# FuxiComputerVision/Nefii

Measured on AMD Instinct MI355X. Metric: training rays/sec (Step-2 material opt), higher is better.
Workload: dtype f16x3; 1 GPU; cfg3; parallelism=dp1, trace_tier=True, bracket_staged_eval=False, split_fp8=False, step_graph=False, cycle_batches=4, trace_prefetch=3, nonfinite_steps=0

## Files before the change

### nefii_amd/csrc/nefii_mlp.hip

```cpp
#include "mlp_tile.h"
#include "hip_check.h"

using namespace nefii;

static inline int round32(int v) { return (v + 31) & ~31; }
static inline int pad_hidden(int v) { return v <= 32 ? round32(v) : (v + 63) & ~63; }
extern "C" int nefii_padded_width(int v) { return v < 0 ? NEFII_E_ARG : pad_hidden(v); }

extern "C" int nefii_abi_version(void) { return NEFII_ABI_VERSION; }

struct PackGeom {
    int n_out, k_in, kx, ke, n_pad, x_src0, x_len, e_src0, e_len;
    float scale;
    __device__ __forceinline__ int src_col(int kk) const {
        if (kk < kx) return kk < x_len ? x_src0 + kk : -1;
        const int e = kk - kx;
        return e < e_len ? e_src0 + e : -1;
    }
    __device__ __forceinline__ float at(const float *__restrict__ W, int n, int kk) const {
        const int c = src_col(kk);
        return (n < n_out && c >= 0) ? W[(size_t)n * k_in + c] * scale : 0.f;
    }
};

// ... 611 lines not shown
    for (int j = 0; j < 8; ++j) v[j] = (_Float16)0.f;
    if (s16 < ((m.layer[l].k_x + m.layer[l].k_e) >> 4)) v = w[(((size_t)s16 * 16 + t) * 2 + part) * 64 + lane_src];
    dst[((size_t)wave * G + g) * 256 + threadIdx.x] = v;
}

__global__ void pack_mlp_stream_bwd_kernel(nefii_mlp m, half8 *__restrict__ dst, int G) {
    const int g = blockIdx.x, wave = blockIdx.y;
    int l = m.n_layers - 1, s = g;
    while (s >= mb_units(m.layer[l])) s -= mb_units(m.layer[l]), --l;
    const nefii_layer &L = m.layer[l];
    const half8 *wb = reinterpret_cast<const half8 *>(L.w_bwd_f16x3);
    const int KT = (L.k_x + L.k_e) >> 5;
    const int f = threadIdx.x >> 6, lane = threadIdx.x & 63, kg = lane >> 4;
    const int kk = 64 * wave + 16 * f + (lane & 15);
    const int s16 = 2 * s + (kg >> 1), t = kk >> 5, lane_src = (kk & 31) + 32 * (kg & 1);
    half8 v;
    for (int j = 0; j < 8; ++j) v[j] = (_Float16)0.f;
    if (s16 < (L.n_pad >> 4)) v = wb[(((size_t)s16 * KT + t) * 2) * 64 + lane_src];
    dst[((size_t)wave * G + g) * 256 + threadIdx.x] = v;
}

extern "C" int nefii_pack_mlp_stream(const nefii_mlp *h_mlp, void *w_stream, void *stream) {
    if (!h_mlp || !w_stream) return NEFII_E_ARG;
    if (nefii_mlp_stream_bytes(h_mlp) == 0) return NEFII_E_UNSUPPORTED;
    const int G = mstream_units(h_mlp);
    hipLaunchKernelGGL(pack_mlp_stream_kernel, dim3(G, 8), dim3(256), 0, (hipStream_t)stream, *h_mlp, (half8 *)w_stream, G);
    HIP_CHECK_LAUNCH();
    const int Gb = mstream_units_bwd(h_mlp);
    if (Gb > 0) {
        hipLaunchKernelGGL(pack_mlp_stream_bwd_kernel, dim3(Gb, 8), dim3(256), 0, (hipStream_t)stream, *h_mlp,
                           (half8 *)w_stream + (size_t)8 * G * 256, Gb);
        HIP_CHECK_LAUNCH();
    }
    return 0;
}

template <int QT, int EW, bool H16>
__global__ __launch_bounds__(512, 2) void mlp_forward16q_kernel(nefii_mlp m, const float *__restrict__ in_a,
                                                               const float *__restrict__ in_b,
                                                               const float *__restrict__ in_c,
                                                               const float *__restrict__ feat, int64_t n,
                                                               float *__restrict__ out, int out_stride,
                                                               float *__restrict__ hidden_out, int hid_stride,
                                                               void *__restrict__ stash_v, int stash_stride,
                                                               float *__restrict__ z_last, _Float16 *__restrict__ x0_16, int G) {
    NEFII_CLAIM_SIMD_2();
    float *const stash = H16 ? nullptr : static_cast<float *>(stash_v);
    _Float16 *const stash16 = H16 ? static_cast<_Float16 *>(stash_v) : nullptr;
    constexpr int ROWS = 16 * QT, XP = LdsM<QT, EW>::XP, EP = 512, NW = 8, NJ = 4 * QT, RT = (QT + 1) / 2;
    __shared__ LdsM<QT, EW> lds;
    __shared__ float raw[ROWS * 9];
    const int tid = threadIdx.x;
    const int wave = __builtin_amdgcn_readfirstlane(tid >> 6), lane = tid & 63;
    const int NH = m.n_layers - 1;
    const float inv_scale = 1.f / (W16_SCALE * A16_SCALE);
    const int64_t n_tiles = (n + ROWS - 1) / ROWS;
    {
        uint32_t *z = reinterpret_cast<uint32_t *>(&lds);
        for (int i = tid; i < (int)(sizeof(lds) / 4); i += 512) z[i] = 0u;
    }
    P16<8>::Stage b[4];
    PCursor cur;
    cur.bytes = (unsigned)G * 4096;
    cur.base = reinterpret_cast<const half8 *>(m.w_stream) + (size_t)wave * G * 256 + lane;
    cur.off = 0;
#pragma unroll
    for (int u = 0; u < 3; ++u) pload<8>(b[u], cur);
    const int boff = 64 * wave + lane;
    const _Float16 *qh0 = lds.Xh + (lane & 15) * XP + 8 * (lane >> 4), *ql0 = lds.Xl + (lane & 15) * XP + 8 * (lane >> 4);
    const int w0 = enc_width(m.enc_freqs[0]), w1 = enc_width(m.enc_freqs[1]), w2 = enc_width(m.enc_freqs[2]);
    const int F = m.feat_width, kx0 = m.layer[0].k_x;
    __syncthreads();
    for (int64_t tile = blockIdx.x; tile < n_tiles; tile += gridDim.x) {
        const int64_t base = tile * ROWS;
        for (int i = tid; i < ROWS * 9; i += 512) {
            const int p = i / 9, c = i - 9 * p, which = c / 3;
            const float *src = which == 0 ? in_a : (which == 1 ? in_b : in_c);
            int64_t idx = base + p;
            if (idx >= n) idx = n - 1;
            raw[i] = (src && m.enc_freqs[which] >= 0) ? src[idx * 3 + (c - 3 * which)] : 0.f;
        }
        if (feat && F == kx0 && (F & 3) == 0 && (reinterpret_cast<uintptr_t>(feat) & 15) == 0) {
            const int q4 = kx0 >> 2;
            for (int i = tid; i < ROWS * q4; i += 512) {
                const int p = i / q4, f = 4 * (i - p * q4);
                int64_t idx = base + p;
                if (idx >= n) idx = n - 1;
                const float4v v = *reinterpret_cast<const float4v *>(feat + idx * F + f) * A16_SCALE;
                const half4 hi = __builtin_convertvector(v, half4);
                *reinterpret_cast<half4 *>(lds.Xh + p * XP + EP - kx0 + f) = hi;
                *reinterpret_cast<half4 *>(lds.Xl + p * XP + EP - kx0 + f) =
                    __builtin_convertvector(v - __builtin_convertvector(hi, float4v), half4);
            }
        } else {
            for (int i = tid; i < ROWS * kx0; i += 512) {
                const int p = i / kx0, f = i - p * kx0;
                int64_t idx = base + p;
                if (idx >= n) idx = n - 1;
                const float v = (feat && f < F) ? feat[idx * F + f] : 0.f;
                split16a(v, lds.Xh[p * XP + EP - kx0 + f], lds.Xl[p * XP + EP - kx0 + f]);
            }
        }
        float bnext = m.layer[0].bias[boff];
        __syncthreads();
        for (int i = tid; i < ROWS * EW; i += 512) {
            const int p = i / EW, c = i - p * EW;
            float val = 0.f;
            if (c < w0) val = enc_value(raw + p * 9, c);
            else if (c < w0 + w1) val = enc_value(raw + p * 9 + 3, c - w0);
            else if (c < w0 + w1 + w2) val = enc_value(raw + p * 9 + 6, c - w0 - w1);
            split16a(val, lds.Xh[p * XP + EP + c], lds.Xl[p * XP + EP + c]);
        }
        __syncthreads();
        if (H16 && x0_16) {
            const int C = (kx0 + EW) >> 3;
            for (int i = tid; i < ROWS * C; i += 512) {
                const int p = i / C, c = i - p * C;
                if (base + p < n)
                    *reinterpret_cast<half8 *>(x0_16 + (size_t)(base + p) * (kx0 + EW) + 8 * c) =
                        *reinterpret_cast<const half8 *>(lds.Xh + p * XP + EP - kx0 + 8 * c);
            }
        }
        for (int l = 0; l < NH; ++l) {
            const nefii_layer &L = m.layer[l];
            const int units = m_units(L);
            const _Float16 *ah = qh0 + (EP - L.k_x), *al = ql0 + (EP - L.k_x);
            const float *bp = m.layer[l + 1 < NH ? l + 1 : l].bias + boff;
            asm volatile("" ::"s"(units), "v"(ah), "v"(al), "v"(bp));
            __builtin_amdgcn_s_waitcnt(0x0070);
            __builtin_amdgcn_sched_barrier(0);
            const float bvec = bnext;
            f32x4 acc[NJ];
#pragma unroll
            for (int j = 0; j < NJ; ++j)
#pragma unroll
                for (int i = 0; i < 4; ++i) acc[j][i] = 0.f;
            QAct<QT> a[2];
            qload_a<QT, XP>(a[0], ah, al, 0);
            qgemm<QT, 4, XP>(units, b, a, cur, ah, al, acc);
            bnext = *bp;
            __builtin_amdgcn_sched_barrier(0);
            half4 phi[NJ], plo[NJ];
            const int bsrc = __builtin_bit_cast(int, bvec);
            const bool pre_last = hidden_out != nullptr && l == NH - 1;
            auto epilogue = [&](auto actc) {
                constexpr int ACT = decltype(actc)::value;
#pragma unroll
                for (int ft = 0; ft < 4; ++ft) {
                    float4v bs;
#pragma unroll
                    for (int k = 0; k < 4; ++k)
                        bs[k] = __builtin_bit_cast(float, __builtin_amdgcn_ds_bpermute(4 * (16 * ft + 4 * (lane >> 4) + k), bsrc));
                    const int f0 = 64 * wave + 16 * ft + 4 * (lane >> 4);
#pragma unroll
                    for (int qt = 0; qt < QT; ++qt) {
                        const int j = ft * QT + qt;
                        float4v hv;
#pragma unroll
                        for (int k = 0; k < 4; ++k) {
                            const float z = __builtin_fmaf(acc[j][k], inv_scale, bs[k]);
                            hv[k] = ACT == NEFII_ACT_ELU ? elu_fast(z) : act_fwd(z, ACT);
                        }
                        const int64_t row = base + 16 * qt + (lane & 15);
                        if (row < n) {
                            if (stash) *reinterpret_cast<float4v *>(stash + ((size_t)l * n + row) * stash_stride + f0) = hv;
                            if (pre_last) {
#pragma unroll
                                for (int k = 0; k < 4; ++k)
                                    if (f0 + k < L.n_out) hidden_out[(size_t)row * hid_stride + f0 + k] = hv[k];
                            }
                        }
                        const float4v hs = hv * A16_SCALE;
                        const half4 hi = __builtin_convertvector(hs, half4);
                        phi[j] = hi;
                        plo[j] = __builtin_convertvector(hs - __builtin_convertvector(hi, float4v), half4);
// ... 71 lines not shown
            __syncthreads();
        }
    }
}

static int check_mlp16(const nefii_mlp *m, bool bwd) {
    int rc = check_mlp(m, false);
    if (rc) return rc;
    for (int l = 0; l < m->n_layers; ++l) {
        if (!m->layer[l].w_f16x3) return NEFII_E_ARG;
        if (bwd && l > 0 && !m->layer[l].w_bwd_f16x3) return NEFII_E_ARG;
        if ((m->layer[l].k_x | m->layer[l].k_e | m->layer[l].n_pad) & 15) return NEFII_E_SHAPE;
    }
    return 0;
}

static bool mlp_stream_enabled() {
    static const bool v = env_int("NEFII_MLP_STREAM", 1) != 0;
    return v;
}
static bool mlp_streams_both_ways(const nefii_mlp *m) {
    return m->w_stream && mlp_stream_enabled() && mstream_shape(m) && mstream_units_bwd(m) > 0;
}
static dim3 stream_grid(int64_t n) {
    const int64_t t = (n + 63) / 64;
    return dim3((int)(t < 256 ? t : 256));
}

template <bool H16>
static int launch_forward16q(const nefii_mlp *h_mlp, const float *in_a, const float *in_b, const float *in_c, const float *feat,
                             int64_t n, float *out, int out_stride, float *hidden_out, int hid_stride, void *stash,
                             int stash_stride, float *z_last, void *x0_16, void *stream) {
    const auto kernel = mstream_shape(h_mlp) == 64 ? mlp_forward16q_kernel<4, 64, H16> : mlp_forward16q_kernel<4, 96, H16>;
    hipLaunchKernelGGL(kernel, stream_grid(n), dim3(512), 0, (hipStream_t)stream, *h_mlp, in_a, in_b, in_c, feat, n, out,
                       out_stride, hidden_out, hid_stride, stash, stash_stride, z_last, (_Float16 *)x0_16, mstream_units(h_mlp));
    HIP_CHECK_LAUNCH();
    return 0;
}

extern "C" int nefii_mlp_forward_f16(const nefii_mlp *h_mlp, const float *in_a, const float *in_b, const float *in_c,
                                     const float *feat, int64_t n, float *out, int out_stride, float *hidden_out,
                                     int hid_stride, float *stash, int stash_stride, int single_pass, void *stream) {
    int rc = check_mlp16(h_mlp, false);
    if (rc) return rc;
    if (n <= 0) return 0;
    if (!out) return NEFII_E_ARG;
    const int64_t n_tiles = (n + TILE - 1) / TILE;
    if (!single_pass && h_mlp->w_stream && mlp_stream_enabled() && mstream_shape(h_mlp))
        return launch_forward16q<false>(h_mlp, in_a, in_b, in_c, feat, n, out, out_stride, hidden_out, hid_stride, stash,
                                        stash_stride, nullptr, nullptr, stream);
    if (single_pass)
        hipLaunchKernelGGL(mlp_forward16_kernel<true>, dim3(grid_for(n_tiles, 1)), dim3(WG), 0, (hipStream_t)stream, *h_mlp,
                           in_a, in_b, in_c, feat, n, out, out_stride, hidden_out, hid_stride, stash, stash_stride);
    else
        hipLaunchKernelGGL(mlp_forward16_kernel<false>, dim3(grid_for(n_tiles, 1)), dim3(WG), 0, (hipStream_t)stream, *h_mlp,
                           in_a, in_b, in_c, feat, n, out, out_stride, hidden_out, hid_stride, stash, stash_stride);
    HIP_CHECK_LAUNCH();
    return 0;
}

extern "C" int nefii_mlp_h16_supported(const nefii_mlp *h_mlp) {
    if (!h_mlp || check_mlp16(h_mlp, true)) return 0;
    return mlp_streams_both_ways(h_mlp);
}

extern "C" int nefii_mlp_x0_width(const nefii_mlp *h_mlp) {
    if (!nefii_mlp_h16_supported(h_mlp)) return 0;
    return h_mlp->layer[0].k_x + mstream_shape(h_mlp);
}

extern "C" int nefii_mlp_forward_f16h(const nefii_mlp *h_mlp, const float *in_a, const float *in_b, const float *in_c,
                                      const float *feat, int64_t n, float *out, int out_stride, float *hidden_out,
                                      int hid_stride, void *stash16, int stash_stride, float *z_last, void *x0_16,
                                      void *stream) {
    int rc = check_mlp16(h_mlp, false);
    if (rc) return rc;
    if (!nefii_mlp_h16_supported(h_mlp)) return NEFII_E_SHAPE;
    if (n <= 0) return 0;
    if (!out || !stash16 || !z_last || (stash_stride & 3)) return NEFII_E_ARG;
    return launch_forward16q<true>(h_mlp, in_a, in_b, in_c, feat, n, out, out_stride, hidden_out, hid_stride, stash16,
                                   stash_stride, z_last, x0_16, stream);
}

__global__ void grad_scale_kernel(const float *__restrict__ d, int64_t count, float *__restrict__ scale) {
    __shared__ float wmax[16];
    float mx = 0.f;
    for (int64_t i = threadIdx.x; i < count; i += blockDim.x) {
        const float v = fabsf(d[i]);
        mx = (v < 3.0e38f && v > mx) ? v : mx;
    }
#pragma unroll
    for (int o = 32; o > 0; o >>= 1) mx = fmaxf(mx, __shfl_xor(mx, o));
    if ((threadIdx.x & 63) == 0) wmax[threadIdx.x >> 6] = mx;
    __syncthreads();
    if (threadIdx.x == 0) {
        for (int w = 1; w < (int)(blockDim.x >> 6); ++w) mx = fmaxf(mx, wmax[w]);
        float s = 1.f;
        if (mx > 0.f) {
            int e;
            frexpf(mx, &e);
            e = 8 - e;
            e = e < -40 ? -40 : (e > 60 ? 60 : e);
            s = ldexpf(1.f, e);
        }
        scale[0] = s;
    }
}

__global__ void grad_scale_head_kernel(const float *__restrict__ d, int out_stride, const float *__restrict__ pre, int pre_stride,
                                       int64_t n, int n_out, int head, float *__restrict__ scale) {
    __shared__ float wmax[16];
    float mx = 0.f;
    const int64_t count = n * n_out;
    for (int64_t i = threadIdx.x; i < count; i += blockDim.x) {
        const int64_t p = i / n_out;
        const int c = (int)(i - p * n_out);
        const float dv = d[p * out_stride + c], z = pre[p * pre_stride + c];
        const float v = fabsf(dv);
        const float hv = fabsf(dv * head_bwd_from_out(head_fwd(z, head), z, head)) * 0.125f;
        mx = (v < 3.0e38f && v > mx) ? v : mx;
        mx = (hv < 3.0e38f && hv > mx) ? hv : mx;
    }
#pragma unroll
    for (int o = 32; o > 0; o >>= 1) mx = fmaxf(mx, __shfl_xor(mx, o));
    if ((threadIdx.x & 63) == 0) wmax[threadIdx.x >> 6] = mx;
    __syncthreads();
    if (threadIdx.x == 0) {
        for (int w = 1; w < (int)(blockDim.x >> 6); ++w) mx = fmaxf(mx, wmax[w]);
        float s = 1.f;
        if (mx > 0.f) {
            int e;
            frexpf(mx, &e);
            e = 8 - e;
            e = e < -40 ? -40 : (e > 60 ? 60 : e);
            s = ldexpf(1.f, e);
        }
        scale[0] = s;
    }
}

extern "C" int nefii_mlp_grad_scale_head(const float *d_out, int out_stride, const float *pre, int pre_stride, int64_t n,
                                         int n_out, int head, float *scale, void *stream) {
    if (!d_out || !pre || !scale || n < 0 || n_out < 1 || out_stride < n_out || pre_stride < n_out) return NEFII_E_ARG;
    if (head < NEFII_HEAD_NONE || head > NEFII_HEAD_RELU_INIT) return NEFII_E_ARG;
    hipLaunchKernelGGL(grad_scale_head_kernel, dim3(1), dim3(1024), 0, (hipStream_t)stream, d_out, out_stride, pre, pre_stride, n,
                       n_out, head, scale);
    HIP_CHECK_LAUNCH();
    return 0;
}

extern "C" int nefii_mlp_grad_scale(const float *d_out, int64_t count, float *scale, void *stream) {
    if (!d_out || !scale || count < 0) return NEFII_E_ARG;
    hipLaunchKernelGGL(grad_scale_kernel, dim3(1), dim3(1024), 0, (hipStream_t)stream, d_out, count, scale);
    HIP_CHECK_LAUNCH();
    return 0;
}

__global__ __launch_bounds__(256, 2) void mlp_backward16_kernel(nefii_mlp m, const float *__restrict__ d_out,
                                                                int out_stride, const float *__restrict__ stash,
                                                                int stash_stride, int64_t n, float *__restrict__ dz,
                                                                int dz_stride, const float *__restrict__ scale) {
    __shared__ _Float16 Xh[TILE * XS16];
    const int tid = threadIdx.x;
    const int Lm1 = m.n_layers - 1;
    const float S = scale[0];
    const float inv = 1.f / (W16_SCALE * S);
    const int64_t n_tiles = (n + TILE - 1) / TILE;
    for (int64_t tile = blockIdx.x; tile < n_tiles; tile += gridDim.x) {
        const int64_t base = tile * TILE;
        {
            const nefii_layer &L = m.layer[Lm1];
            for (int i = tid; i < TILE * L.n_pad; i += WG) {
                const int p = i / L.n_pad, c = i - p * L.n_pad;
                float v = 0.f;
                if (base + p < n && c < L.n_out) {
                    const float pre = stash[((size_t)Lm1 * n + base + p) * stash_stride + c];
                    const float y = head_fwd(pre, m.head);
                    v = d_out[(size_t)(base + p) * out_stride + c] * head_bwd_from_out(y, pre, m.head);
                }
                Xh[p * XS16 + c] = (_Float16)(v * S);
                if (base + p < n) dz[((size_t)Lm1 * n + base + p) * dz_stride + c] = v;
            }
        }
        __syncthreads();
        for (int l = Lm1; l >= 1; --l) {
            const nefii_layer &L = m.layer[l];
            f32x16 acc[4];
            const int wave = __builtin_amdgcn_readfirstlane(tid >> 6), lane = tid & 63;
            const int NTs = (L.k_x + L.k_e) >> 5, ntc = L.k_x >> 5;
            int ntw = (ntc - wave + 3) >> 2;
            if (ntw < 0) ntw = 0;
            zero_acc(acc);
            gemm_block16<true>(Xh, Xh, XS16, L.n_pad >> 4, reinterpret_cast<const half8 *>(L.w_bwd_f16x3), NTs, wave, lane,
                               ntw, acc);
            __syncthreads();
            NEFII_ACT_SWITCH(m.act, {
                NEFII_FOR_ACC(acc, ntw, {
                    const bool live = (base + row) < n;
                    float v = 0.f;
                    if (live) {
                        const float hprev = stash[((size_t)(l - 1) * n + base + row) * stash_stride + col];
                        v = val * inv * act_bwd_from_out(hprev, ACT);
                        dz[((size_t)(l - 1) * n + base + row) * dz_stride + col] = v;
                    }
                    Xh[row * XS16 + col] = (_Float16)(v * S);
                })
            })
            __syncthreads();
        }
    }
}

template <bool H16>
__global__ __launch_bounds__(512, 2) void mlp_backward16s_kernel(nefii_mlp m, const float *__restrict__ d_out, int out_stride,
                                                                const void *__restrict__ stash_v, int stash_stride,
                                                                const float *__restrict__ z_last, int64_t n,
                                                                void *__restrict__ dz_v, int dz_stride,
                                                                const float *__restrict__ scale, size_t stream_off, int G) {
    NEFII_CLAIM_SIMD_2();
    const float *const stash = static_cast<const float *>(stash_v);
    const _Float16 *const stash16 = static_cast<const _Float16 *>(stash_v);
    float *const dz = static_cast<float *>(dz_v);
    _Float16 *const dz16 = static_cast<_Float16 *>(dz_v);
    constexpr int QT = 4, FT = 4, ROWS = 64, XP = QGeo<4>::XP, NJ = FT * QT;
    __shared__ LdsS<4, ROWS> lds;
    const int tid = threadIdx.x;
    const int wave = __builtin_amdgcn_readfirstlane(tid >> 6), lane = tid & 63;
    const int Lm1 = m.n_layers - 1;
    const float S = scale[0];
    const float inv = 1.f / (W16_SCALE * S);
    const int64_t n_tiles = (n + ROWS - 1) / ROWS;
    {
        uint32_t *z = reinterpret_cast<uint32_t *>(&lds);
        for (int i = tid; i < (int)(sizeof(lds) / 4); i += 512) z[i] = 0u;
    }
    SStage<4> b[4];
    PCursor cur;
    cur.bytes = (unsigned)G * 4096;
    cur.base = reinterpret_cast<const half8 *>(m.w_stream) + stream_off + (size_t)wave * G * 256 + lane;
    cur.off = 0;
#pragma unroll
    for (int u = 0; u < 3; ++u) sload<4>(b[u], cur);
    const _Float16 *qh0 = lds.Xh + (lane & 15) * XP + 8 * (lane >> 4);
    __syncthreads();
    for (int64_t tile = blockIdx.x; tile < n_tiles; tile += gridDim.x) {
        const int64_t base = tile * ROWS;
        {
            const nefii_layer &L = m.layer[Lm1];
            const int kpad = mb_units(L) * 32;
            for (int i = tid; i < ROWS * kpad; i += 512) {
                const int p = i / kpad, c = i - p * kpad;
                float v = 0.f;
                if (base + p < n && c < L.n_pad) {
                    if (c < L.n_out) {
                        const float pre = H16 ? z_last[(size_t)(base + p) * 8 + c]
                                              : stash[((size_t)Lm1 * n + base + p) * stash_stride + c];
                        const float y = head_fwd(pre, m.head);
                        v = d_out[(size_t)(base + p) * out_stride + c] * head_bwd_from_out(y, pre, m.head);
                    }
                    if (H16) dz16[((size_t)Lm1 * n + base + p) * dz_stride + c] = (_Float16)(v * S);
                    else dz[((size_t)Lm1 * n + base + p) * dz_stride + c] = v;
                }
                lds.Xh[p * XP + c] = (_Float16)(v * S);
            }
        }
        __syncthreads();
        for (int l = Lm1; l >= 1; --l) {
            const nefii_layer &L = m.layer[l];
            const int units = mb_units(L);
            asm volatile("" ::"s"(units));
            __builtin_amdgcn_s_waitcnt(0x0070);
            __builtin_amdgcn_sched_barrier(0);
            f32x4 acc[NJ];
#pragma unroll
            for (int j = 0; j < NJ; ++j)
#pragma unroll
                for (int i = 0; i < 4; ++i) acc[j][i] = 0.f;
            SAct<QT> a[2];
            sload_a<QT, XP>(a[0], qh0, 0);
            sgemm<QT, FT, true>(units, b, a, cur, qh0, acc);
            half4 phi[NJ];
            const float *sp = stash + (size_t)(l - 1) * n * stash_stride;
            float *dp = dz + (size_t)(l - 1) * n * dz_stride;
            const _Float16 *sp16 = stash16 + (size_t)(l - 1) * n * stash_stride;
            _Float16 *dp16 = dz16 + (size_t)(l - 1) * n * dz_stride;
            auto epilogue = [&](auto actc) {
                constexpr int ACT = decltype(actc)::value;
#pragma unroll
                for (int ft = 0; ft < FT; ++ft) {
                    const int f0 = 64 * wave + 16 * ft + 4 * (lane >> 4);
#pragma unroll
                    for (int qt = 0; qt < QT; ++qt) {
                        const int j = ft * QT + qt;
                        const int64_t row = base + 16 * qt + (lane & 15);
                        float4v v = {0.f, 0.f, 0.f, 0.f};
                        if (row < n) {
                            float4v h;
                            if (H16)
                                h = __builtin_convertvector(*reinterpret_cast<const half4 *>(sp16 + (size_t)row * stash_stride + f0),
                                                            float4v) * (1.f / A16_SCALE);
                            else
                                h = *reinterpret_cast<const float4v *>(sp + (size_t)row * stash_stride + f0);
#pragma unroll
                            for (int k = 0; k < 4; ++k) v[k] = acc[j][k] * inv * act_bwd_from_out(h[k], ACT);
                            if (!H16) *reinterpret_cast<float4v *>(dp + (size_t)row * dz_stride + f0) = v;
                        }
                        phi[j] = __builtin_convertvector(v * S, half4);
                        if (H16 && row < n) *reinterpret_cast<half4 *>(dp16 + (size_t)row * dz_stride + f0) = phi[j];
                    }
                }
            };
            if (m.act == NEFII_ACT_RELU)
                epilogue(std::integral_constant<int, NEFII_ACT_RELU>{});
            else if (m.act == NEFII_ACT_ELU)
                epilogue(std::integral_constant<int, NEFII_ACT_ELU>{});
            else
                epilogue(std::integral_constant<int, NEFII_ACT_SOFTPLUS100>{});
            __syncthreads();
#pragma unroll
            for (int ft = 0; ft < FT; ++ft) {
                const int f0 = 64 * wave + 16 * ft + 4 * (lane >> 4);
#pragma unroll
                for (int qt = 0; qt < QT; ++qt)
                    *reinterpret_cast<half4 *>(lds.Xh + (16 * qt + (lane & 15)) * XP + f0) = phi[ft * QT + qt];
            }
            __syncthreads();
        }
    }
}

template <bool H16>
static int launch_backward16s(const nefii_mlp *h_mlp, const float *d_out, int out_stride, const void *stash, int stash_stride,
                              const float *z_last, int64_t n, void *dz, int dz_stride, const float *scale, void *stream) {
    hipLaunchKernelGGL(mlp_backward16s_kernel<H16>, stream_grid(n), dim3(512), 0, (hipStream_t)stream, *h_mlp, d_out, out_stride,
                       stash, stash_stride, z_last, n, dz, dz_stride, scale, (size_t)8 * mstream_units(h_mlp) * 256,
                       mstream_units_bwd(h_mlp));
    HIP_CHECK_LAUNCH();
    return 0;
}

extern "C" int nefii_mlp_backward_f16(const nefii_mlp *h_mlp, const float *d_out, int out_stride, const float *stash,
                                      int stash_stride, int64_t n, float *dz, int dz_stride, const float *scale,
                                      void *stream) {
    int rc = check_mlp16(h_mlp, true);
    if (rc) return rc;
    if (n <= 0) return 0;
    if (!d_out || !stash || !dz || !scale) return NEFII_E_ARG;
    if (mlp_streams_both_ways(h_mlp) && (stash_stride & 3) == 0 && (dz_stride & 3) == 0)
        return launch_backward16s<false>(h_mlp, d_out, out_stride, stash, stash_stride, nullptr, n, dz, dz_stride, scale, stream);
    const int64_t n_tiles = (n + TILE - 1) / TILE;
    hipLaunchKernelGGL(mlp_backward16_kernel, dim3(grid_for(n_tiles, 2)), dim3(WG), 0, (hipStream_t)stream, *h_mlp, d_out,
                       out_stride, stash, stash_stride, n, dz, dz_stride, scale);
    HIP_CHECK_LAUNCH();
    return 0;
}

extern "C" int nefii_mlp_backward_f16h(const nefii_mlp *h_mlp, const float *d_out, int out_stride, const void *stash16,
                                       int stash_stride, const float *z_last, int64_t n, void *dz16, int dz_stride,
                                       const float *scale, void *stream) {
    int rc = check_mlp16(h_mlp, true);
    if (rc) return rc;
    if (!nefii_mlp_h16_supported(h_mlp)) return NEFII_E_SHAPE;
    if (n <= 0) return 0;
    if (!d_out || !stash16 || !z_last || !dz16 || !scale || (stash_stride & 3) || (dz_stride & 3)) return NEFII_E_ARG;
    return launch_backward16s<true>(h_mlp, d_out, out_stride, stash16, stash_stride, z_last, n, dz16, dz_stride, scale, stream);
}

template <bool DZ16, bool X16>
__device__ __forceinline__ void wgrad16_body(const void *__restrict__ dz_v, int dz_stride, const void *__restrict__ x_v,
                                             int x_stride, int64_t P, int n_out, int k_in, float scale,
                                             const float *__restrict__ gscale, float *__restrict__ dW, float *__restrict__ db,
                                             int atomic, int bx, int by, int bz, int gz) {
    const float *const dz = static_cast<const float *>(dz_v), *const x = static_cast<const float *>(x_v);
    const _Float16 *const dz16 = static_cast<const _Float16 *>(dz_v), *const x16 = static_cast<const _Float16 *>(x_v);
    const int wave = threadIdx.x >> 6, lane = threadIdx.x & 63;
    const int i = lane & 31, h = lane >> 5;
    const int n0 = bx * 64 + (wave & 1) * 32;
    const int k0 = by * 256 + (wave >> 1) * 128;
    const int64_t chunk = ((P + gz - 1) / gz + 15) & ~(int64_t)15;
    const int64_t p_begin = (int64_t)bz * chunk;
    const int64_t p_end = p_begin + chunk < P ? p_begin + chunk : P;
    const float S = gscale[0];
    f32x16 acc[4];
    zero_acc(acc);
    const bool n_ok = (n0 + i) < n_out;
    bool k_ok[4];
#pragma unroll
    for (int t = 0; t < 4; ++t) k_ok[t] = (k0 + 32 * t + i) < k_in;
    float bsum = 0.f;
    if (n0 < n_out && k0 < k_in) {
        const int nc = n_ok ? n0 + i : n_out - 1;
// ... 122 lines not shown
                    for (int e = 0; e < 8; ++e) a[e] = na + e < n_out ? a[e] : (_Float16)0;
                }
                ha[u] = pr < p_end ? a : hzero;
            }
        } else {
#pragma unroll
            for (int u = 0; u < 4; ++u) {
                const int64_t pr = pb + r8 + 8 * u;
                const int64_t pc = pr < p_end ? pr : p_end - 1;
                float4v a = {0.f, 0.f, 0.f, 0.f};
                if (n_in) {
                    a = *reinterpret_cast<const float4v *>(dz + pc * dz_stride + na);
                } else {
#pragma unroll
                    for (int e = 0; e < 4; ++e) a[e] = dz[pc * dz_stride + (na + e < n_out ? na + e : n_out - 1)];
#pragma unroll
                    for (int e = 0; e < 4; ++e) a[e] = na + e < n_out ? a[e] : 0.f;
                }
                ra[u] = pr < p_end ? a : float4v{0.f, 0.f, 0.f, 0.f};
            }
        }
        if (X16) {
#pragma unroll
            for (int u = 0; u < 2; ++u) {
                const int64_t pr = pb + r16 + 16 * u;
                const int64_t pc = pr < p_end ? pr : p_end - 1;
                half8 b = hzero;
                if (XVEC && k_in_ok) {
                    b = *reinterpret_cast<const half8 *>(x16 + pc * x_stride + ka);
                } else {
#pragma unroll
                    for (int e = 0; e < 8; ++e) b[e] = x16[pc * x_stride + (ka + e < k_in ? ka + e : k_in - 1)];
#pragma unroll
                    for (int e = 0; e < 8; ++e) b[e] = ka + e < k_in ? b[e] : (_Float16)0;
                }
                hb[u] = pr < p_end ? b : hzero;
            }
        } else {
#pragma unroll
            for (int u = 0; u < 4; ++u) {
                const int64_t pr = pb + r8 + 8 * u;
                const int64_t pc = pr < p_end ? pr : p_end - 1;
                float4v b = {0.f, 0.f, 0.f, 0.f};
                if (XVEC && k_in_ok) {
                    b = *reinterpret_cast<const float4v *>(x + pc * x_stride + ka);
                } else {
#pragma unroll
                    for (int e = 0; e < 4; ++e) b[e] = x[pc * x_stride + (ka + e < k_in ? ka + e : k_in - 1)];
#pragma unroll
                    for (int e = 0; e < 4; ++e) b[e] = ka + e < k_in ? b[e] : 0.f;
                }
                rb[u] = pr < p_end ? b : float4v{0.f, 0.f, 0.f, 0.f};
            }
        }
    };
    auto stage = [&](int buf) {
        if (DZ16) {
#pragma unroll
            for (int u = 0; u < 2; ++u) {
#pragma unroll
                for (int e = 0; e < 8; ++e) bsum[e] += (float)ha[u][e];
                *reinterpret_cast<half8 *>(&A[buf][(r16 + 16 * u) * WG2_STRIDE + 8 * c8]) = ha[u];
            }
        } else {
#pragma unroll
            for (int u = 0; u < 4; ++u) {
#pragma unroll
                for (int e = 0; e < 4; ++e) bsum[e] += ra[u][e];
                *reinterpret_cast<half4 *>(&A[buf][(r8 + 8 * u) * WG2_STRIDE + 4 * c4]) = __builtin_convertvector(ra[u] * S, half4);
            }
        }
        if (X16) {
#pragma unroll
            for (int u = 0; u < 2; ++u) *reinterpret_cast<half8 *>(&B[buf][(r16 + 16 * u) * WG2_STRIDE + 8 * c8]) = hb[u];
        } else {
#pragma unroll
            for (int u = 0; u < 4; ++u)
                *reinterpret_cast<half4 *>(&B[buf][(r8 + 8 * u) * WG2_STRIDE + 4 * c4]) = __builtin_convertvector(rb[u], half4);
        }
    };
    f32x16 acc[4];
    zero_acc(acc);
    const int an = 64 * (wave & 1), bk = 64 * (wave >> 1);
    fetch(p_begin);
    stage(0);
    __syncthreads();
    int buf = 0;
    for (int64_t pb = p_begin; pb < p_end; pb += WG2_ROWS) {
        const bool more = pb + WG2_ROWS < p_end;
        if (more) fetch(pb + WG2_ROWS);
#pragma unroll
        for (int ks = 0; ks < 2; ++ks) {
            half8 af[2], bf[2];
#pragma unroll
            for (int t = 0; t < 2; ++t) {
                af[t] = wg2_fragment(A[buf], an + 32 * t, 16 * ks, lane);
                bf[t] = wg2_fragment(B[buf], bk + 32 * t, 16 * ks, lane);
            }
#pragma unroll
            for (int t = 0; t < 2; ++t)
#pragma unroll
                for (int v = 0; v < 2; ++v)
                    acc[2 * t + v] = __builtin_amdgcn_mfma_f32_32x32x16_f16(af[t], bf[v], acc[2 * t + v], 0, 0, 0);
        }
        if (more) stage(buf ^ 1);
        __syncthreads();
        buf ^= 1;
    }
    const float os = scale / S * (X16 ? 1.f / A16_SCALE : 1.f);
    const int i = lane & 31, h = lane >> 5;
#pragma unroll
    for (int t = 0; t < 2; ++t)
#pragma unroll
        for (int v = 0; v < 2; ++v)
#pragma unroll
            for (int r = 0; r < 16; ++r) {
                const int nn = n0 + an + 32 * t + (r & 3) + 8 * (r >> 2) + 4 * h, k = k0 + bk + 32 * v + i;
                if (nn < n_out && k < k_in) atomicAdd(&dW[(size_t)nn * k_in + k], acc[2 * t + v][r] * os);
            }
    if (db && tk == 0) {
        __syncthreads();
        float *red = reinterpret_cast<float *>(&A[0][0]);
        if (DZ16) {
#pragma unroll
            for (int e = 0; e < 8; ++e) red[r16 * 128 + 8 * c8 + e] = bsum[e];
        } else {
#pragma unroll
            for (int e = 0; e < 4; ++e) red[r8 * 128 + 4 * c4 + e] = bsum[e];
        }
        __syncthreads();
        if (tid < 128 && n0 + tid < n_out) {
            float sum = 0.f;
#pragma unroll
            for (int g = 0; g < (DZ16 ? 16 : 8); ++g) sum += red[g * 128 + tid];
            atomicAdd(&db[n0 + tid], DZ16 ? sum / S : sum);
        }
    }
}

template <bool XVEC, bool DZ16, bool X16>
__global__ __launch_bounds__(256, 2) void mlp_wgrad16t_kernel(const void *__restrict__ dz_v, int dz_stride,
                                                              const void *__restrict__ x_v, int x_stride, int64_t P, int n_out,
                                                              int k_in, float scale, const float *__restrict__ gscale,
                                                              float *__restrict__ dW, float *__restrict__ db, int splits,
                                                              int tiles_n, int tiles_k) {
    wgrad16t_body<XVEC, DZ16, X16>(dz_v, dz_stride, x_v, x_stride, P, n_out, k_in, scale, gscale, dW, db, splits, tiles_n, tiles_k,
                                   blockIdx.x);
}

struct WgradBatch {
    nefii_wgrad_item it[NEFII_MAX_WGRAD_ITEMS];
    unsigned first[NEFII_MAX_WGRAD_ITEMS + 1];
    int aux0[NEFII_MAX_WGRAD_ITEMS], aux1[NEFII_MAX_WGRAD_ITEMS], aux2[NEFII_MAX_WGRAD_ITEMS];
    int n;
};
__device__ __forceinline__ int wgrad_batch_item(const WgradBatch &b, unsigned bid) {
    int i = 0;
    while (i + 1 < b.n && bid >= b.first[i + 1]) ++i;
    return __builtin_amdgcn_readfirstlane(i);
}
template <bool XVEC, bool X16>
__global__ __launch_bounds__(256, 2) void mlp_wgrad16t_batch_kernel(WgradBatch b, int64_t P, const float *__restrict__ gscale) {
    const int i = wgrad_batch_item(b, blockIdx.x);
    const nefii_wgrad_item &w = b.it[i];
    wgrad16t_body<XVEC, true, X16>(w.dz16, w.dz_stride, w.x, w.x_stride, P, w.n_out, w.k_in, w.scale, gscale, w.dW, w.db, b.aux0[i],
                                   b.aux1[i], b.aux2[i], blockIdx.x - b.first[i]);
}
template <bool X16>
__global__ __launch_bounds__(256) void mlp_wgrad16_batch_kernel(WgradBatch b, int64_t P, const float *__restrict__ gscale) {
    const int i = wgrad_batch_item(b, blockIdx.x);
    const nefii_wgrad_item &w = b.it[i];
    const int local = blockIdx.x - b.first[i], gx = b.aux0[i], gy = b.aux1[i], gz = b.aux2[i];
    wgrad16_body<true, X16>(w.dz16, w.dz_stride, w.x, w.x_stride, P, w.n_out, w.k_in, w.scale, gscale, w.dW, w.db, gz > 1 ? 1 : 0,
                            local % gx, (local / gx) % gy, local / (gx * gy), gz);
}
__global__ void zero_fill_batch_kernel(WgradBatch b) {
    const int i = wgrad_batch_item(b, blockIdx.x);
    const nefii_wgrad_item &w = b.it[i];
    const size_t e = (size_t)(blockIdx.x - b.first[i]) * blockDim.x + threadIdx.x, nw = (size_t)w.n_out * w.k_in;
    if (e < nw) w.dW[e] = 0.f;
    else if (w.db && e - nw < (size_t)w.n_out) w.db[e - nw] = 0.f;
}

static bool wgrad_tr_enabled() {
    static const bool v = env_int("NEFII_WGRAD_TR", 1) != 0;
    return v;
}

struct WgradPlan {
    bool blocked, xvec, needs_zero_fill;
// ... 359 lines not shown
```

Measured before the change: 2.009 million rays/s.

## Batch loads in MLP kernels, parallelize grad-scale, deepen weight-grad prefetch

Several independent changes. The feature-load loop issues four vector loads before converting them. The grad-scale reductions become a multi-block reduction using atomicMax plus clear and finish kernels when the input is large. The backward head and activation epilogues are restructured to issue stash loads up front with clamped rows. The weight-gradient GEMM gains a two-stage register prefetch path for full 128x128 fp16 tiles. Together these aim to expose more memory-level parallelism and to stop a single block from serializing the reduction, at the cost of more registers and extra kernel launches.

```diff
diff --git a/nefii_amd/csrc/nefii_mlp.hip b/nefii_amd/csrc/nefii_mlp.hip
--- a/nefii_amd/csrc/nefii_mlp.hip
+++ b/nefii_amd/csrc/nefii_mlp.hip
@@ -717,15 +717,29 @@
         }
         if (feat && F == kx0 && (F & 3) == 0 && (reinterpret_cast<uintptr_t>(feat) & 15) == 0) {
             const int q4 = kx0 >> 2;
-            for (int i = tid; i < ROWS * q4; i += 512) {
-                const int p = i / q4, f = 4 * (i - p * q4);
-                int64_t idx = base + p;
-                if (idx >= n) idx = n - 1;
-                const float4v v = *reinterpret_cast<const float4v *>(feat + idx * F + f) * A16_SCALE;
-                const half4 hi = __builtin_convertvector(v, half4);
-                *reinterpret_cast<half4 *>(lds.Xh + p * XP + EP - kx0 + f) = hi;
-                *reinterpret_cast<half4 *>(lds.Xl + p * XP + EP - kx0 + f) =
-                    __builtin_convertvector(v - __builtin_convertvector(hi, float4v), half4);
+            constexpr int FG = 4;
+            for (int i0 = tid; i0 < ROWS * q4; i0 += FG * 512) {
+                float4v v[FG];
+#pragma unroll
+                for (int u = 0; u < FG; ++u) {
+                    const int i = i0 + u * 512 < ROWS * q4 ? i0 + u * 512 : ROWS * q4 - 1;
+                    const int p = i / q4, f = 4 * (i - p * q4);
+                    int64_t idx = base + p;
+                    if (idx >= n) idx = n - 1;
+                    v[u] = *reinterpret_cast<const float4v *>(feat + idx * F + f);
+                }
+#pragma unroll
+                for (int u = 0; u < FG; ++u) {
+                    const int i = i0 + u * 512;
+                    if (i < ROWS * q4) {
+                        const int p = i / q4, f = 4 * (i - p * q4);
+                        const float4v w = v[u] * A16_SCALE;
+                        const half4 hi = __builtin_convertvector(w, half4);
+                        *reinterpret_cast<half4 *>(lds.Xh + p * XP + EP - kx0 + f) = hi;
+                        *reinterpret_cast<half4 *>(lds.Xl + p * XP + EP - kx0 + f) =
+                            __builtin_convertvector(w - __builtin_convertvector(hi, float4v), half4);
+                    }
+                }
             }
         } else {
             for (int i = tid; i < ROWS * kx0; i += 512) {
@@ -963,6 +977,17 @@
                                    stash_stride, z_last, x0_16, stream);
 }
 
+__device__ __forceinline__ float gs_from_max(float mx) {
+    float s = 1.f;
+    if (mx > 0.f) {
+        int e;
+        frexpf(mx, &e);
+        e = 8 - e;
+        e = e < -40 ? -40 : (e > 60 ? 60 : e);
+        s = ldexpf(1.f, e);
+    }
+    return s;
+}
 __global__ void grad_scale_kernel(const float *__restrict__ d, int64_t count, float *__restrict__ scale) {
     __shared__ float wmax[16];
     float mx = 0.f;
@@ -976,15 +1001,7 @@
     __syncthreads();
     if (threadIdx.x == 0) {
         for (int w = 1; w < (int)(blockDim.x >> 6); ++w) mx = fmaxf(mx, wmax[w]);
-        float s = 1.f;
-        if (mx > 0.f) {
-            int e;
-            frexpf(mx, &e);
-            e = 8 - e;
-            e = e < -40 ? -40 : (e > 60 ? 60 : e);
-            s = ldexpf(1.f, e);
-        }
-        scale[0] = s;
+        scale[0] = gs_from_max(mx);
     }
 }
 
@@ -1008,31 +1025,135 @@
     __syncthreads();
     if (threadIdx.x == 0) {
         for (int w = 1; w < (int)(blockDim.x >> 6); ++w) mx = fmaxf(mx, wmax[w]);
-        float s = 1.f;
-        if (mx > 0.f) {
-            int e;
-            frexpf(mx, &e);
-            e = 8 - e;
-            e = e < -40 ? -40 : (e > 60 ? 60 : e);
-            s = ldexpf(1.f, e);
-        }
-        scale[0] = s;
-    }
+        scale[0] = gs_from_max(mx);
+    }
+}
+
+constexpr int64_t GS_ONE_BLOCK = 65536;
+constexpr int GS_WG = 256, GS_U = 4;
+
+__device__ __forceinline__ float gs_fold(float mx, float v) {
+    return (v < 3.0e38f && v > mx) ? v : mx;
+}
+__device__ __forceinline__ void gs_block_max(float mx, float *__restrict__ scale) {
+    __shared__ float wmax[GS_WG / 64];
+#pragma unroll
+    for (int o = 32; o > 0; o >>= 1) mx = fmaxf(mx, __shfl_xor(mx, o));
+    if ((threadIdx.x & 63) == 0) wmax[threadIdx.x >> 6] = mx;
+    __syncthreads();
+    if (threadIdx.x == 0) {
+#pragma unroll
+        for (int w = 1; w < GS_WG / 64; ++w) mx = fmaxf(mx, wmax[w]);
+        if (mx > 0.f) atomicMax(reinterpret_cast<unsigned *>(scale), __float_as_uint(mx));
+    }
+}
+__global__ void grad_scale_clear_kernel(float *__restrict__ scale) { scale[0] = 0.f; }
+__global__ void grad_scale_finish_kernel(float *__restrict__ scale) { scale[0] = gs_from_max(scale[0]); }
+
+template <bool VEC>
+__global__ __launch_bounds__(GS_WG) void grad_scale_blocks_kernel(const float *__restrict__ d, int64_t count,
+                                                                  float *__restrict__ scale) {
+    float mx = 0.f;
+    const int64_t stride = (int64_t)gridDim.x * GS_WG;
+    const int64_t t = (int64_t)blockIdx.x * GS_WG + threadIdx.x;
+    if (VEC) {
+        const int64_t quads = count >> 2;
+        const float4v *d4 = reinterpret_cast<const float4v *>(d);
+        for (int64_t i = t; i < quads; i += GS_U * stride) {
+            float4v v[GS_U];
+#pragma unroll
+            for (int u = 0; u < GS_U; ++u) {
+                const int64_t k = i + u * stride;
+                v[u] = d4[k < quads ? k : quads - 1];
+            }
+#pragma unroll
+            for (int u = 0; u < GS_U; ++u)
+#pragma unroll
+                for (int e = 0; e < 4; ++e) mx = gs_fold(mx, fabsf(v[u][e]));
+        }
+        if (blockIdx.x == 0 && threadIdx.x < (count & 3)) mx = gs_fold(mx, fabsf(d[(quads << 2) + threadIdx.x]));
+    } else {
+        for (int64_t i = t; i < count; i += GS_U * stride) {
+            float v[GS_U];
+#pragma unroll
+            for (int u = 0; u < GS_U; ++u) {
+                const int64_t k = i + u * stride;
+                v[u] = d[k < count ? k : count - 1];
+            }
+#pragma unroll
+            for (int u = 0; u < GS_U; ++u) mx = gs_fold(mx, fabsf(v[u]));
+        }
+    }
+    gs_block_max(mx, scale);
+}
+
+__global__ __launch_bounds__(GS_WG) void grad_scale_head_blocks_kernel(const float *__restrict__ d, int out_stride,
+                                                                       const float *__restrict__ pre, int pre_stride, int64_t n,
+                                                                       int n_out, int head, float *__restrict__ scale) {
+    float mx = 0.f;
+    const int64_t count = n * n_out;
+    const int64_t stride = (int64_t)gridDim.x * GS_WG;
+    for (int64_t i = (int64_t)blockIdx.x * GS_WG + threadIdx.x; i < count; i += GS_U * stride) {
+        float dv[GS_U], z[GS_U];
+#pragma unroll
+        for (int u = 0; u < GS_U; ++u) {
+            const int64_t k = i + u * stride, kc = k < count ? k : count - 1;
+            const int64_t p = kc / n_out;
+            const int c = (int)(kc - p * n_out);
+            dv[u] = d[p * out_stride + c];
+            z[u] = pre[p * pre_stride + c];
+        }
+#pragma unroll
+        for (int u = 0; u < GS_U; ++u) {
+            mx = gs_fold(mx, fabsf(dv[u]));
+            mx = gs_fold(mx, fabsf(dv[u] * head_bwd_from_out(head_fwd(z[u], head), z[u], head)) * 0.125f);
+        }
+    }
+    gs_block_max(mx, scale);
+}
+
+static int gs_grid(int64_t units) {
+    const int64_t g = (units + (int64_t)GS_WG * GS_U - 1) / ((int64_t)GS_WG * GS_U);
+    return (int)(g < 1 ? 1 : (g > 2048 ? 2048 : g));
 }
 
 extern "C" int nefii_mlp_grad_scale_head(const float *d_out, int out_stride, const float *pre, int pre_stride, int64_t n,
                                          int n_out, int head, float *scale, void *stream) {
     if (!d_out || !pre || !scale || n < 0 || n_out < 1 || out_stride < n_out || pre_stride < n_out) return NEFII_E_ARG;
     if (head < NEFII_HEAD_NONE || head > NEFII_HEAD_RELU_INIT) return NEFII_E_ARG;
-    hipLaunchKernelGGL(grad_scale_head_kernel, dim3(1), dim3(1024), 0, (hipStream_t)stream, d_out, out_stride, pre, pre_stride, n,
-                       n_out, head, scale);
+    hipStream_t st = (hipStream_t)stream;
+    if (n * n_out <= GS_ONE_BLOCK) {
+        hipLaunchKernelGGL(grad_scale_head_kernel, dim3(1), dim3(1024), 0, st, d_out, out_stride, pre, pre_stride, n, n_out, head,
+                           scale);
+        HIP_CHECK_LAUNCH();
+        return 0;
+    }
+    hipLaunchKernelGGL(grad_scale_clear_kernel, dim3(1), dim3(1), 0, st, scale);
+    HIP_CHECK_LAUNCH();
+    hipLaunchKernelGGL(grad_scale_head_blocks_kernel, dim3(gs_grid(n * n_out)), dim3(GS_WG), 0, st, d_out, out_stride, pre,
+                       pre_stride, n, n_out, head, scale);
+    HIP_CHECK_LAUNCH();
+    hipLaunchKernelGGL(grad_scale_finish_kernel, dim3(1), dim3(1), 0, st, scale);
     HIP_CHECK_LAUNCH();
     return 0;
 }
 
 extern "C" int nefii_mlp_grad_scale(const float *d_out, int64_t count, float *scale, void *stream) {
     if (!d_out || !scale || count < 0) return NEFII_E_ARG;
-    hipLaunchKernelGGL(grad_scale_kernel, dim3(1), dim3(1024), 0, (hipStream_t)stream, d_out, count, scale);
+    hipStream_t st = (hipStream_t)stream;
+    if (count <= GS_ONE_BLOCK) {
+        hipLaunchKernelGGL(grad_scale_kernel, dim3(1), dim3(1024), 0, st, d_out, count, scale);
+        HIP_CHECK_LAUNCH();
+        return 0;
+    }
+    hipLaunchKernelGGL(grad_scale_clear_kernel, dim3(1), dim3(1), 0, st, scale);
+    HIP_CHECK_LAUNCH();
+    if ((reinterpret_cast<uintptr_t>(d_out) & 15) == 0)
+        hipLaunchKernelGGL(grad_scale_blocks_kernel<true>, dim3(gs_grid(count >> 2)), dim3(GS_WG), 0, st, d_out, count, scale);
+    else
+        hipLaunchKernelGGL(grad_scale_blocks_kernel<false>, dim3(gs_grid(count)), dim3(GS_WG), 0, st, d_out, count, scale);
+    HIP_CHECK_LAUNCH();
+    hipLaunchKernelGGL(grad_scale_finish_kernel, dim3(1), dim3(1), 0, st, scale);
     HIP_CHECK_LAUNCH();
     return 0;
 }
@@ -1129,18 +1250,29 @@
         {
             const nefii_layer &L = m.layer[Lm1];
             const int kpad = mb_units(L) * 32;
+            const int n_out = L.n_out;
             for (int i = tid; i < ROWS * kpad; i += 512) {
                 const int p = i / kpad, c = i - p * kpad;
-                float v = 0.f;
-                if (base + p < n && c < L.n_pad) {
-                    if (c < L.n_out) {
-                        const float pre = H16 ? z_last[(size_t)(base + p) * 8 + c]
-                                              : stash[((size_t)Lm1 * n + base + p) * stash_stride + c];
-                        const float y = head_fwd(pre, m.head);
-                        v = d_out[(size_t)(base + p) * out_stride + c] * head_bwd_from_out(y, pre, m.head);
+                if (c >= n_out) {
+                    lds.Xh[p * XP + c] = (_Float16)0.f;
+                    if (base + p < n && c < L.n_pad) {
+                        if (H16) dz16[((size_t)Lm1 * n + base + p) * dz_stride + c] = (_Float16)0.f;
+                        else dz[((size_t)Lm1 * n + base + p) * dz_stride + c] = 0.f;
                     }
-                    if (H16) dz16[((size_t)Lm1 * n + base + p) * dz_stride + c] = (_Float16)(v * S);
-                    else dz[((size_t)Lm1 * n + base + p) * dz_stride + c] = v;
+                }
+            }
+            for (int i = tid; i < ROWS * n_out; i += 512) {
+                const int p = i / n_out, c = i - p * n_out;
+                const bool live = base + p < n;
+                const int64_t rc = live ? base + p : n - 1;
+                const float pre = H16 ? z_last[(size_t)rc * 8 + c] : stash[((size_t)Lm1 * n + rc) * stash_stride + c];
+                const float dv = d_out[(size_t)rc * out_stride + c];
+                const float y = head_fwd(pre, m.head);
+                const float g = dv * head_bwd_from_out(y, pre, m.head);
+                const float v = live ? g : 0.f;
+                if (live) {
+                    if (H16) dz16[((size_t)Lm1 * n + rc) * dz_stride + c] = (_Float16)(v * S);
+                    else dz[((size_t)Lm1 * n + rc) * dz_stride + c] = v;
                 }
                 lds.Xh[p * XP + c] = (_Float16)(v * S);
             }
@@ -1165,29 +1297,61 @@
             float *dp = dz + (size_t)(l - 1) * n * dz_stride;
             const _Float16 *sp16 = stash16 + (size_t)(l - 1) * n * stash_stride;
             _Float16 *dp16 = dz16 + (size_t)(l - 1) * n * dz_stride;
+            bool live[QT];
+            size_t srow[QT];
+#pragma unroll
+            for (int qt = 0; qt < QT; ++qt) {
+                const int64_t row = base + 16 * qt + (lane & 15);
+                live[qt] = row < n;
+                srow[qt] = (size_t)(live[qt] ? row : n - 1) * stash_stride + 64 * wave + 4 * (lane >> 4);
+            }
             auto epilogue = [&](auto actc) {
                 constexpr int ACT = decltype(actc)::value;
-#pragma unroll
-                for (int ft = 0; ft < FT; ++ft) {
-                    const int f0 = 64 * wave + 16 * ft + 4 * (lane >> 4);
-#pragma unroll
-                    for (int qt = 0; qt < QT; ++qt) {
-                        const int j = ft * QT + qt;
-                        const int64_t row = base + 16 * qt + (lane & 15);
-                        float4v v = {0.f, 0.f, 0.f, 0.f};
-                        if (row < n) {
-                            float4v h;
-                            if (H16)
-                                h = __builtin_convertvector(*reinterpret_cast<const half4 *>(sp16 + (size_t)row * stash_stride + f0),
-                                                            float4v) * (1.f / A16_SCALE);
-                            else
-                                h = *reinterpret_cast<const float4v *>(sp + (size_t)row * stash_stride + f0);
-#pragma unroll
-                            for (int k = 0; k < 4; ++k) v[k] = acc[j][k] * inv * act_bwd_from_out(h[k], ACT);
-                            if (!H16) *reinterpret_cast<float4v *>(dp + (size_t)row * dz_stride + f0) = v;
+                if constexpr (H16) {
+                    half4 hs[NJ];
+#pragma unroll
+                    for (int ft = 0; ft < FT; ++ft)
+#pragma unroll
+                        for (int qt = 0; qt < QT; ++qt)
+                            hs[ft * QT + qt] = *reinterpret_cast<const half4 *>(sp16 + srow[qt] + 16 * ft);
+#pragma unroll
+                    for (int ft = 0; ft < FT; ++ft)
+#pragma unroll
+                        for (int qt = 0; qt < QT; ++qt) {
+                            const int j = ft * QT + qt;
+                            const float4v h = __builtin_convertvector(hs[j], float4v) * (1.f / A16_SCALE);
+                            float4v v;
+#pragma unroll
+                            for (int k = 0; k < 4; ++k) v[k] = live[qt] ? acc[j][k] * inv * act_bwd_from_out(h[k], ACT) : 0.f;
+                            phi[j] = __builtin_convertvector(v * S, half4);
                         }
-                        phi[j] = __builtin_convertvector(v * S, half4);
-                        if (H16 && row < n) *reinterpret_cast<half4 *>(dp16 + (size_t)row * dz_stride + f0) = phi[j];
+#pragma unroll
+                    for (int qt = 0; qt < QT; ++qt)
+                        if (live[qt]) {
+                            _Float16 *drow = dp16 + (size_t)(base + 16 * qt + (lane & 15)) * dz_stride + 64 * wave + 4 * (lane >> 4);
+#pragma unroll
+                            for (int ft = 0; ft < FT; ++ft) *reinterpret_cast<half4 *>(drow + 16 * ft) = phi[ft * QT + qt];
+                        }
+                } else {
+#pragma unroll
+                    for (int ft = 0; ft < FT; ++ft) {
+                        float4v hs[QT];
+#pragma unroll
+                        for (int qt = 0; qt < QT; ++qt) hs[qt] = *reinterpret_cast<const float4v *>(sp + srow[qt] + 16 * ft);
+#pragma unroll
+                        for (int qt = 0; qt < QT; ++qt) {
+                            const int j = ft * QT + qt;
+                            float4v v;
+#pragma unroll
+                            for (int k = 0; k < 4; ++k) v[k] = live[qt] ? acc[j][k] * inv * act_bwd_from_out(hs[qt][k], ACT) : 0.f;
+                            hs[qt] = v;
+                            phi[j] = __builtin_convertvector(v * S, half4);
+                        }
+#pragma unroll
+                        for (int qt = 0; qt < QT; ++qt)
+                            if (live[qt])
+                                *reinterpret_cast<float4v *>(dp + (size_t)(base + 16 * qt + (lane & 15)) * dz_stride + 64 * wave +
+                                                             4 * (lane >> 4) + 16 * ft) = hs[qt];
                     }
                 }
             };
@@ -1476,13 +1640,7 @@
     f32x16 acc[4];
     zero_acc(acc);
     const int an = 64 * (wave & 1), bk = 64 * (wave >> 1);
-    fetch(p_begin);
-    stage(0);
-    __syncthreads();
-    int buf = 0;
-    for (int64_t pb = p_begin; pb < p_end; pb += WG2_ROWS) {
-        const bool more = pb + WG2_ROWS < p_end;
-        if (more) fetch(pb + WG2_ROWS);
+    auto products = [&](int buf) {
 #pragma unroll
         for (int ks = 0; ks < 2; ++ks) {
             half8 af[2], bf[2];
@@ -1497,9 +1655,64 @@
                 for (int v = 0; v < 2; ++v)
                     acc[2 * t + v] = __builtin_amdgcn_mfma_f32_32x32x16_f16(af[t], bf[v], acc[2 * t + v], 0, 0, 0);
         }
-        if (more) stage(buf ^ 1);
+    };
+    bool done = false;
+    if constexpr (XVEC && DZ16 && X16) {
+        if (n0 + 128 <= n_out && k0 + 128 <= k_in) {
+            half8 qa[2][2], qb[2][2];
+            auto fetch2 = [&](int s, int64_t pb) {
+#pragma unroll
+                for (int u = 0; u < 2; ++u) {
+                    const int64_t pr = pb + r16 + 16 * u;
+                    const int64_t pc = pr < p_end ? pr : p_end - 1;
+                    qa[s][u] = *reinterpret_cast<const half8 *>(dz16 + pc * dz_stride + na);
+                    qb[s][u] = *reinterpret_cast<const half8 *>(x16 + pc * x_stride + ka);
+                }
+            };
+            auto stage2 = [&](int s, int buf, int64_t pb) {
+#pragma unroll
+                for (int u = 0; u < 2; ++u) {
+                    const bool in = pb + r16 + 16 * u < p_end;
+                    const half8 a = in ? qa[s][u] : hzero;
+#pragma unroll
+                    for (int e = 0; e < 8; ++e) bsum[e] += (float)a[e];
+                    *reinterpret_cast<half8 *>(&A[buf][(r16 + 16 * u) * WG2_STRIDE + 8 * c8]) = a;
+                    *reinterpret_cast<half8 *>(&B[buf][(r16 + 16 * u) * WG2_STRIDE + 8 * c8]) = in ? qb[s][u] : hzero;
+                }
+            };
+            fetch2(0, p_begin);
+            stage2(0, 0, p_begin);
+            fetch2(0, p_begin + WG2_ROWS);
+            fetch2(1, p_begin + 2 * WG2_ROWS);
+            __syncthreads();
+            for (int64_t pb = p_begin; !done; pb += 2 * WG2_ROWS) {
+#pragma unroll
+                for (int j = 0; j < 2; ++j) {
+                    if (done) continue;
+                    products(j);
+                    done = pb + (j + 1) * WG2_ROWS >= p_end;
+                    if (!done) {
+                        stage2(j, j ^ 1, pb + (j + 1) * WG2_ROWS);
+                        fetch2(j, pb + (j + 3) * WG2_ROWS);
+                        __syncthreads();
+                    }
+                }
+            }
+        }
+    }
+    if (!done) {
+        fetch(p_begin);
+        stage(0);
         __syncthreads();
-        buf ^= 1;
+        int buf = 0;
+        for (int64_t pb = p_begin; pb < p_end; pb += WG2_ROWS) {
+            const bool more = pb + WG2_ROWS < p_end;
+            if (more) fetch(pb + WG2_ROWS);
+            products(buf);
+            if (more) stage(buf ^ 1);
+            __syncthreads();
+            buf ^= 1;
+        }
     }
     const float os = scale / S * (X16 ? 1.f / A16_SCALE : 1.f);
     const int i = lane & 31, h = lane >> 5;
```

Measured after the change: 2.040 million rays/s, median of 6. 1.5% higher.
